# FederatedAI/FATE-LLM

Measured on AMD Instinct MI355X. Metric: GB/s param buffer reconstructed from (seed,scalar) list, device-resident, higher is better.
Workload: dtype bf16

## Files before the change

fate-llm_amd/csrc/fks_device.hip:

```cpp
#include <hip/hip_runtime.h>
#include <hip/hip_bf16.h>

#include <atomic>
#include <type_traits>
#include <mutex>

#include "fks_internal.h"
#include "fks_bitslice.h"
#define FKS_HD __device__ __forceinline__
#include "fks_libm.h"

constexpr int kDbMinWaves = 4;
constexpr int kZrUnroll = 2;
constexpr int kSm2MinWaves = 8;
constexpr int kBsFence = 8;
#ifndef FKS_BS_LAG
#define FKS_BS_LAG 36
#endif
#ifndef FKS_F32_SEED_PAIRS
#define FKS_F32_SEED_PAIRS 0
#endif
#ifndef FKS_LOG_INTMASK
#define FKS_LOG_INTMASK 1
#endif
#ifndef FKS_F32_TRIM
#define FKS_F32_TRIM 1
#endif

namespace fks {
namespace {

__device__ __forceinline__ uint32_t mt_twist(uint32_t u, uint32_t v) {
  return (((u & 0x80000000u) | (v & 0x7fffffffu)) >> 1) ^ ((v & 1u) ? kMatrixA : 0u);
}

constexpr unsigned kXorAnd = 0x78;
constexpr unsigned kXorMask = 0x28;
constexpr unsigned kXorNotAnd = 0xD2;

__device__ __forceinline__ uint32_t mt_temper(uint32_t y) {
  y ^= (y >> 11);
  y = __builtin_amdgcn_bitop3_b32(y, y << 7, 0x9d2c5680u, kXorAnd);
  y = __builtin_amdgcn_bitop3_b32(y, y << 15, 0xefc60000u, kXorAnd);
  y ^= (y >> 18);
  return y;
}


typedef __bf16 bf16x2_t __attribute__((ext_vector_type(2)));
typedef float f32x2_t __attribute__((ext_vector_type(2)));
__device__ __forceinline__ float rbf_cvt(float x) {
  const f32x2_t v = {0.0f, x};
  return __builtin_bit_cast(float, __builtin_convertvector(v, bf16x2_t));
}
__device__ __forceinline__ float rbf(float x) { return rbf_cvt(x); }
__device__ __forceinline__ float rhf(float x) {
  asm volatile("" : "+v"(x));
  return static_cast<float>(static_cast<_Float16>(x));
}

__device__ __forceinline__ uint32_t swap_adjacent(uint32_t v) {
  return (uint32_t)__builtin_amdgcn_mov_dpp((int)v, 0xB1, 0xF, 0xF, false);
}

__device__ __forceinline__ float cephes_logf(float x) {
#if FKS_LOG_INTMASK
  const uint32_t xb0 = __float_as_uint(x);
  const uint32_t xb = (xb0 & ~0x7f800000u) | 0x3f000000u;
  const int32_t m = (int32_t)(xb - 0x3F3504F3u) >> 31;
  const float e = (float)((int32_t)(xb0 >> 23) - 126 + m);
  const float tmp = __uint_as_float(xb & (uint32_t)m);
  x = __uint_as_float(xb) - 1.0f;
#else
  int32_t imm0 = (int32_t)(__float_as_uint(x) >> 23);
  x = __uint_as_float((__float_as_uint(x) & ~0x7f800000u) | 0x3f000000u);
  imm0 -= 0x7f;
  float e = (float)imm0;
  e = e + 1.0f;
  const bool mask = x < 0.707106781186547524f;
  const float tmp = mask ? x : 0.0f;
  x = x - 1.0f;
  e = e - (mask ? 1.0f : 0.0f);
#endif
  x = x + tmp;
  const float z = x * x;
  float y = 7.0376836292E-2f;
  y = __fmaf_rn(y, x, -1.1514610310E-1f);
  y = __fmaf_rn(y, x, 1.1676998740E-1f);
  y = __fmaf_rn(y, x, -1.2420140846E-1f);
  y = __fmaf_rn(y, x, +1.4249322787E-1f);
  y = __fmaf_rn(y, x, -1.6668057665E-1f);
  y = __fmaf_rn(y, x, +2.0000714765E-1f);
  y = __fmaf_rn(y, x, -2.4999993993E-1f);
  y = __fmaf_rn(y, x, +3.3333331174E-1f);
  y = y * x;
  y = __fmaf_rn(y, z, e * -2.12194440e-4f);
  y = __fmaf_rn(-z, 0.5f, y);
  x = x + y;
  x = __fmaf_rn(e, 0.693359375f, x);
  return x;
}


template <int DT>
struct Traits;

typedef __attribute__((address_space(1))) float gf32;
typedef __attribute__((address_space(1))) uint16_t gu16;
typedef __attribute__((address_space(1))) _Float16 gf16;

typedef __attribute__((address_space(1))) uint32_t gu32;

typedef __attribute__((address_space(1))) uint64_t gu64;

template <>
struct Traits<FKS_F32> {
  typedef uint64_t Pair;
  __device__ static Pair load_pair(uint64_t a) { return *reinterpret_cast<const gu64*>(a); }
  __device__ static void store_pair(uint64_t a, Pair v) { *reinterpret_cast<gu64*>(a) = v; }
  __device__ static uint32_t lo(Pair v) { return (uint32_t)v; }
  __device__ static uint32_t hi(Pair v) { return (uint32_t)(v >> 32); }
  __device__ static Pair pack(uint32_t l, uint32_t h) { return (uint64_t)l | ((uint64_t)h << 32); }
  __device__ static uint32_t bits(float v) { return __float_as_uint(v); }
  __device__ static uint32_t load_raw(uint64_t p, int64_t i) { return reinterpret_cast<const gu32*>(p)[i]; }
  __device__ static float cvt(uint32_t r) { return __uint_as_float(r); }
  __device__ static float load(uint64_t p, int64_t i) { return reinterpret_cast<const gf32*>(p)[i]; }
  __device__ static void store(uint64_t p, int64_t i, float v) { reinterpret_cast<gf32*>(p)[i] = v; }
  __device__ static float rnd(float x) { return x; }
};

template <>
struct Traits<FKS_BF16> {
  typedef uint32_t Pair;
  __device__ static Pair load_pair(uint64_t a) { return *reinterpret_cast<const gu32*>(a); }
  __device__ static void store_pair(uint64_t a, Pair v) { *reinterpret_cast<gu32*>(a) = v; }
  __device__ static uint32_t lo(Pair v) { return v & 0xffffu; }
  __device__ static uint32_t hi(Pair v) { return v >> 16; }
  __device__ static Pair pack(uint32_t l, uint32_t h) { return (l & 0xffffu) | (h << 16); }
  __device__ static uint32_t bits(float v) { return __float_as_uint(v) >> 16; }
  __device__ static uint32_t load_raw(uint64_t p, int64_t i) { return reinterpret_cast<const gu16*>(p)[i]; }
  __device__ static float cvt(uint32_t r) { return __uint_as_float(r << 16); }
  __device__ static float load(uint64_t p, int64_t i) {
    return __uint_as_float((uint32_t)reinterpret_cast<const gu16*>(p)[i] << 16);
  }
  __device__ static void store(uint64_t p, int64_t i, float v) {
    reinterpret_cast<gu16*>(p)[i] = (uint16_t)(__float_as_uint(v) >> 16);
  }
  __device__ static float rnd(float x) { return rbf(x); }
};

template <>
struct Traits<FKS_F16> {
  typedef uint32_t Pair;
  __device__ static Pair load_pair(uint64_t a) { return *reinterpret_cast<const gu32*>(a); }
  __device__ static void store_pair(uint64_t a, Pair v) { *reinterpret_cast<gu32*>(a) = v; }
  __device__ static uint32_t lo(Pair v) { return v & 0xffffu; }
  __device__ static uint32_t hi(Pair v) { return v >> 16; }
  __device__ static Pair pack(uint32_t l, uint32_t h) { return (l & 0xffffu) | (h << 16); }
  __device__ static uint32_t bits(float v) { return __builtin_bit_cast(uint16_t, static_cast<_Float16>(v)); }
  __device__ static uint32_t load_raw(uint64_t p, int64_t i) { return reinterpret_cast<const gu16*>(p)[i]; }
  __device__ static float cvt(uint32_t r) { return static_cast<float>(__builtin_bit_cast(_Float16, (uint16_t)r)); }
  __device__ static float load(uint64_t p, int64_t i) { return static_cast<float>(reinterpret_cast<const gf16*>(p)[i]); }
  __device__ static void store(uint64_t p, int64_t i, float v) { reinterpret_cast<gf16*>(p)[i] = static_cast<_Float16>(v); }
  __device__ static float rnd(float x) { return rhf(x); }
};

template <>
struct Traits<kDtF32Libm> : Traits<FKS_F32> {};
constexpr bool is_f32(int dt) { return dt == FKS_F32 || dt == kDtF32Libm; }

template <int DT>
__device__ __forceinline__ float apply_one(float p, float z, float g, float lr, float wd, bool has_wd, int mode,
                                           float ps, bool upd = true) {
  using TR = Traits<DT>;
  if (mode == kModeDelta) return __fmaf_rn(g, z, p);
  if (mode == kModePerturb || mode == kModePerturbUpdate) {
    p = TR::rnd(p + TR::rnd(ps * z));
    if (mode == kModePerturb || !upd) return p;
  }
  if (mode == kModeUpdate || mode == kModePerturbUpdate) {
    const float gz = TR::rnd(g * z);
    const float t2 = TR::rnd(gz + TR::rnd(wd * p));
    const float t = has_wd ? t2 : gz;
    return TR::rnd(p - TR::rnd(lr * t));
  }
  return z;
}

template <int DT>
__device__ __forceinline__ float dev_value_g(const float* v) {
  const float g = __int_as_float(__builtin_amdgcn_readfirstlane(__float_as_int(v[0])));
  return is_f32(DT) ? g : Traits<DT>::rnd(g);
}
__device__ __forceinline__ bool dev_value_apply(const float* v) {
  return __int_as_float(__builtin_amdgcn_readfirstlane(__float_as_int(v[1]))) != 0.0f;
}

constexpr int kJumpXOff = 3;

__device__ __forceinline__ void jump_quad_step10(uint32_t (&acc)[10], const uint32_t (&w)[13], uint32_t code) {
  asm volatile(
      "s_bitcmp1_b32 %[c], 3\n"
      "s_cbranch_scc1 .Lqb3k8x%=\n"
      "s_bitcmp1_b32 %[c], 2\n"
      "s_cbranch_scc1 .Lqb2k4x%=\n"
      "s_bitcmp1_b32 %[c], 1\n"
      "s_cbranch_scc1 .Lqb1k2x%=\n"
      "s_bitcmp1_b32 %[c], 0\n"
      "s_cbranch_scc1 .Lqb0k1x%=\n"
      "s_branch .Lqendx%=\n"
      ".Lqb0k1x%=:\n"
      "v_xor_b32 %[a0], %[a0], %[w0]\n"
      "v_xor_b32 %[a1], %[a1], %[w1]\n"
      "v_xor_b32 %[a2], %[a2], %[w2]\n"
      "v_xor_b32 %[a3], %[a3], %[w3]\n"
      "v_xor_b32 %[a4], %[a4], %[w4]\n"
      "v_xor_b32 %[a5], %[a5], %[w5]\n"
      "v_xor_b32 %[a6], %[a6], %[w6]\n"
      "v_xor_b32 %[a7], %[a7], %[w7]\n"
      "v_xor_b32 %[a8], %[a8], %[w8]\n"
      "v_xor_b32 %[a9], %[a9], %[w9]\n"
      "s_branch .Lqendx%=\n"
      ".Lqb1k2x%=:\n"
      "s_bitcmp1_b32 %[c], 0\n"
      "s_cbranch_scc1 .Lqb0k3x%=\n"
      "v_xor_b32 %[a0], %[a0], %[w1]\n"
      "v_xor_b32 %[a1], %[a1], %[w2]\n"
      "v_xor_b32 %[a2], %[a2], %[w3]\n"
      "v_xor_b32 %[a3], %[a3], %[w4]\n"
      "v_xor_b32 %[a4], %[a4], %[w5]\n"
      "v_xor_b32 %[a5], %[a5], %[w6]\n"
      "v_xor_b32 %[a6], %[a6], %[w7]\n"
      "v_xor_b32 %[a7], %[a7], %[w8]\n"
      "v_xor_b32 %[a8], %[a8], %[w9]\n"
      "v_xor_b32 %[a9], %[a9], %[w10]\n"
      "s_branch .Lqendx%=\n"
      ".Lqb0k3x%=:\n"
      "v_bitop3_b32 %[a0], %[a0], %[w0], %[w1] bitop3:0x96\n"
      "v_bitop3_b32 %[a1], %[a1], %[w1], %[w2] bitop3:0x96\n"
      "v_bitop3_b32 %[a2], %[a2], %[w2], %[w3] bitop3:0x96\n"
      "v_bitop3_b32 %[a3], %[a3], %[w3], %[w4] bitop3:0x96\n"
      "v_bitop3_b32 %[a4], %[a4], %[w4], %[w5] bitop3:0x96\n"
      "v_bitop3_b32 %[a5], %[a5], %[w5], %[w6] bitop3:0x96\n"
      "v_bitop3_b32 %[a6], %[a6], %[w6], %[w7] bitop3:0x96\n"
      "v_bitop3_b32 %[a7], %[a7], %[w7], %[w8] bitop3:0x96\n"
      "v_bitop3_b32 %[a8], %[a8], %[w8], %[w9] bitop3:0x96\n"
      "v_bitop3_b32 %[a9], %[a9], %[w9], %[w10] bitop3:0x96\n"
      "s_branch .Lqendx%=\n"
      ".Lqb2k4x%=:\n"
      "s_bitcmp1_b32 %[c], 1\n"
      "s_cbranch_scc1 .Lqb1k6x%=\n"
      "s_bitcmp1_b32 %[c], 0\n"
      "s_cbranch_scc1 .Lqb0k5x%=\n"
      "v_xor_b32 %[a0], %[a0], %[w2]\n"
      "v_xor_b32 %[a1], %[a1], %[w3]\n"
      "v_xor_b32 %[a2], %[a2], %[w4]\n"
      "v_xor_b32 %[a3], %[a3], %[w5]\n"
      "v_xor_b32 %[a4], %[a4], %[w6]\n"
      "v_xor_b32 %[a5], %[a5], %[w7]\n"
      "v_xor_b32 %[a6], %[a6], %[w8]\n"
      "v_xor_b32 %[a7], %[a7], %[w9]\n"
      "v_xor_b32 %[a8], %[a8], %[w10]\n"
      "v_xor_b32 %[a9], %[a9], %[w11]\n"
      "s_branch .Lqendx%=\n"
      ".Lqb0k5x%=:\n"
      "v_bitop3_b32 %[a0], %[a0], %[w0], %[w2] bitop3:0x96\n"
      "v_bitop3_b32 %[a1], %[a1], %[w1], %[w3] bitop3:0x96\n"
      "v_bitop3_b32 %[a2], %[a2], %[w2], %[w4] bitop3:0x96\n"
      "v_bitop3_b32 %[a3], %[a3], %[w3], %[w5] bitop3:0x96\n"
      "v_bitop3_b32 %[a4], %[a4], %[w4], %[w6] bitop3:0x96\n"
      "v_bitop3_b32 %[a5], %[a5], %[w5], %[w7] bitop3:0x96\n"
      "v_bitop3_b32 %[a6], %[a6], %[w6], %[w8] bitop3:0x96\n"
      "v_bitop3_b32 %[a7], %[a7], %[w7], %[w9] bitop3:0x96\n"
      "v_bitop3_b32 %[a8], %[a8], %[w8], %[w10] bitop3:0x96\n"
      "v_bitop3_b32 %[a9], %[a9], %[w9], %[w11] bitop3:0x96\n"
      "s_branch .Lqendx%=\n"
      ".Lqb1k6x%=:\n"
      "s_bitcmp1_b32 %[c], 0\n"
      "s_cbranch_scc1 .Lqb0k7x%=\n"
      "v_bitop3_b32 %[a0], %[a0], %[w1], %[w2] bitop3:0x96\n"
      "v_bitop3_b32 %[a1], %[a1], %[w2], %[w3] bitop3:0x96\n"
      "v_bitop3_b32 %[a2], %[a2], %[w3], %[w4] bitop3:0x96\n"
      "v_bitop3_b32 %[a3], %[a3], %[w4], %[w5] bitop3:0x96\n"
      "v_bitop3_b32 %[a4], %[a4], %[w5], %[w6] bitop3:0x96\n"
      "v_bitop3_b32 %[a5], %[a5], %[w6], %[w7] bitop3:0x96\n"
      "v_bitop3_b32 %[a6], %[a6], %[w7], %[w8] bitop3:0x96\n"
      "v_bitop3_b32 %[a7], %[a7], %[w8], %[w9] bitop3:0x96\n"
      "v_bitop3_b32 %[a8], %[a8], %[w9], %[w10] bitop3:0x96\n"
      "v_bitop3_b32 %[a9], %[a9], %[w10], %[w11] bitop3:0x96\n"
      "s_branch .Lqendx%=\n"
      ".Lqb0k7x%=:\n"
      "v_bitop3_b32 %[a0], %[a0], %[w0], %[w1] bitop3:0x96\n"
      "v_xor_b32 %[a0], %[a0], %[w2]\n"
      "v_bitop3_b32 %[a1], %[a1], %[w1], %[w2] bitop3:0x96\n"
      "v_xor_b32 %[a1], %[a1], %[w3]\n"
      "v_bitop3_b32 %[a2], %[a2], %[w2], %[w3] bitop3:0x96\n"
      "v_xor_b32 %[a2], %[a2], %[w4]\n"
      "v_bitop3_b32 %[a3], %[a3], %[w3], %[w4] bitop3:0x96\n"
      "v_xor_b32 %[a3], %[a3], %[w5]\n"
      "v_bitop3_b32 %[a4], %[a4], %[w4], %[w5] bitop3:0x96\n"
      "v_xor_b32 %[a4], %[a4], %[w6]\n"
      "v_bitop3_b32 %[a5], %[a5], %[w5], %[w6] bitop3:0x96\n"
      "v_xor_b32 %[a5], %[a5], %[w7]\n"
      "v_bitop3_b32 %[a6], %[a6], %[w6], %[w7] bitop3:0x96\n"
      "v_xor_b32 %[a6], %[a6], %[w8]\n"
      "v_bitop3_b32 %[a7], %[a7], %[w7], %[w8] bitop3:0x96\n"
      "v_xor_b32 %[a7], %[a7], %[w9]\n"
      "v_bitop3_b32 %[a8], %[a8], %[w8], %[w9] bitop3:0x96\n"
      "v_xor_b32 %[a8], %[a8], %[w10]\n"
      "v_bitop3_b32 %[a9], %[a9], %[w9], %[w10] bitop3:0x96\n"
      "v_xor_b32 %[a9], %[a9], %[w11]\n"
      "s_branch .Lqendx%=\n"
      ".Lqb3k8x%=:\n"
      "s_bitcmp1_b32 %[c], 2\n"
      "s_cbranch_scc1 .Lqb2k12x%=\n"
      "s_bitcmp1_b32 %[c], 1\n"
      "s_cbranch_scc1 .Lqb1k10x%=\n"
      "s_bitcmp1_b32 %[c], 0\n"
      "s_cbranch_scc1 .Lqb0k9x%=\n"
      "v_xor_b32 %[a0], %[a0], %[w3]\n"
// ... 1168 lines not shown
      u32x2_t w0, w1;
      w0.x = w.x;
      w0.y = w.y;
      w1.x = w.z;
      w1.y = w.w;
      zab = temper_pair_u8x8(w0);
      zcd = temper_pair_u8x8(w1);
      a.zidx[((size_t)(b0 + t - a.zlo)) * kZidxPerBlock + q] =
          (zab.x >> 3) | (zab.y << 5) | (zcd.x << 13) | (zcd.y << 21);
    }
    {
      if (sl.fast) {
        run(buf_c, sl.r0, sl.r1, u_lr, u_wd, u_wdf, u_ps);
        ST::store_pair(sl.base + joff, sl.r0);
        ST::store_pair(sl.base + joff + 8 * kEs, sl.r1);
      } else {
        const int64_t s1 = (int64_t)kMtN * (b0 + t) + j;
        int cc = sl.cur;
        bool in = false;
        DevSeg sg;
        while (cc < a.nsegs) {
          sg = a.segs[cc];
          if (s1 < sg.start + sg.numel) { in = s1 >= sg.start; break; }
          cc++;
        }
        if (in) {
          const uint64_t addr = sg.ptr + (uint64_t)(s1 - sg.start) * kEs;
          Pair r0 = 0, r1 = 0;
          if (MODE != kModeWriteZ) {
            r0 = ST::load_pair(addr);
            r1 = ST::load_pair(addr + 8 * kEs);
          }
          run(buf_c, r0, r1, sg.lr, sg.wd, (sg.flags & FKS_HAS_WD) != 0, sg.ps);
          ST::store_pair(addr, r0);
          ST::store_pair(addr + 8 * kEs, r1);
        }
      }
    }
    __syncthreads();
  };

  Slot s0 = fetch(0);
  *reinterpret_cast<volatile uint32_t*>(a.sink + 1) = 0u;
  for (int t = 0; t < nblk; t += 2) {
    Slot s1 = fetch(t + 1 < nblk ? t + 1 : t);
    block(std::integral_constant<int, 0>{}, s0, t);
    if (t + 1 >= nblk) break;
    s0 = fetch(t + 2 < nblk ? t + 2 : t + 1);
    block(std::integral_constant<int, 1>{}, s1, t + 1);
  }
}

constexpr int kZrThreads = 256;
typedef __attribute__((address_space(1))) u32x4_t gu32x4_t;
__device__ __forceinline__ u32x4_t gload4(uint64_t addr) { return *reinterpret_cast<const gu32x4_t*>(addr); }
__device__ __forceinline__ void gstore4(uint64_t addr, u32x4_t v) { *reinterpret_cast<gu32x4_t*>(addr) = v; }
constexpr int kZrTile = kZrThreads * 8;

template <int MODE>
__global__ __launch_bounds__(kZrThreads) void fks_zreplay_kernel(ApplyArgs a) {
  extern __shared__ __attribute__((aligned(16))) uint32_t lds32[];
  if ((uint32_t)(size_t)(lds_u32_t*)lds32 != 0u) __builtin_trap();
  const int tid = threadIdx.x;
  const int c = blockIdx.x;
  for (int i = tid; i < 256; i += kZrThreads) {
    reinterpret_cast<float*>(lds32)[i] = c_tab_bf16[i];
    reinterpret_cast<float*>(lds32)[256 + i] = c_tab_bf16[256 + i];
    reinterpret_cast<float*>(lds32)[512 + i] = c_tab_bf16[512 + i];
  }
  __syncthreads();
  const int64_t p0 = (int64_t)kMtN * a.chunk_block[0] + (int64_t)c * kZrTile;
  const int64_t p1 = (int64_t)kMtN * a.chunk_block[a.nchunks];
  const int64_t tstep = (int64_t)gridDim.x * kZrTile;
  const int64_t zbase = (int64_t)kMtN * a.zlo;
  const uint64_t zb = (uint64_t)(uintptr_t)a.zidx;
  float g = rflf(a.g[0]);
  bool upd = true;
  if (MODE == kModePerturbUpdate && a.gdev) {
    g = dev_value_g<FKS_BF16>(a.gdev);
    upd = dev_value_apply(a.gdev);
  }
  const uint32_t half = (uint32_t)tid & 1u;
  const uint32_t cs_tab = half ? 2048u : 1024u;

  int cur = 0;
  {
    int lo = 0, hi = a.nsegs;
    while (lo < hi) {
      const int mid = (lo + hi) >> 1;
      const DevSeg& sm = a.segs[mid];
      if ((int64_t)rfl64((uint64_t)(sm.start + sm.numel)) <= p0) lo = mid + 1; else hi = mid;
    }
    cur = lo;
  }
  auto chain = [&](u32x4_t pv, u32x4_t rec, float lr, float wd, bool wdf, float ps) __attribute__((always_inline)) -> u32x4_t {
    const uint32_t w[4] = {pv.x, pv.y, pv.z, pv.w};
    const uint32_t r[4] = {rec.x, rec.y, rec.z, rec.w};
    uint32_t o[4];
#pragma unroll
    for (int m = 0; m < 4; m++) {
      const uint32_t ri = r[m];
      const float ra = lds_f32((ri << 2) & 0x3FCu), rb = lds_f32((ri >> 14) & 0x3FCu);
      const float ca = lds_f32(cs_tab + ((ri >> 6) & 0x3FCu)), cb = lds_f32(cs_tab + ((ri >> 22) & 0x3FCu));
      const f32x2_t rr = {ra, rb}, cc = {ca, cb}, zero = {0.0f, 0.0f};
      const f32x2_t z = rnd2<FKS_BF16>(__builtin_elementwise_fma(rr, cc, zero));
      f32x2_t pe = {__uint_as_float(w[m] << 16), __uint_as_float(w[m] & 0xffff0000u)};
      pe = apply_pair<FKS_BF16, MODE>(pe, z, g, lr, wd, wdf, ps, upd);
      o[m] = __builtin_amdgcn_perm(__float_as_uint(pe.y), __float_as_uint(pe.x), 0x07060302u);
    }
    const u32x4_t out = {o[0], o[1], o[2], o[3]};
    return out;
  };
  const u32x4_t zero4 = {0u, 0u, 0u, 0u};
  struct ZSlot { int64_t t0; uint64_t base; float lr, wd, ps; int cur; bool fast, wdf; u32x4_t rec, pv; };
  int64_t seg_st = INT64_MAX, seg_en = INT64_MAX;
  uint64_t seg_ptr = 0;
  float seg_lr = 0.0f, seg_wd = 0.0f, seg_ps = 0.0f;
  bool seg_wdf = false;
  auto load_seg = [&]() __attribute__((always_inline)) {
    if (cur < a.nsegs) {
      const DevSeg& sg = a.segs[cur];
      seg_st = (int64_t)rfl64((uint64_t)sg.start);
      seg_en = seg_st + (int64_t)rfl64((uint64_t)sg.numel);
      seg_ptr = rfl64(sg.ptr);
      seg_lr = rflf(sg.lr);
      seg_wd = rflf(sg.wd);
      seg_ps = rflf(sg.ps);
      seg_wdf = (rfl(sg.flags) & FKS_HAS_WD) != 0;
    } else {
      seg_st = seg_en = INT64_MAX;
    }
  };
  load_seg();
  auto zfetch = [&](int64_t t0) __attribute__((always_inline)) -> ZSlot {
    ZSlot z;
    z.t0 = t0;
    while (seg_en <= t0) {
      cur++;
      load_seg();
    }
    z.cur = cur;
    const int64_t tend = t0 + kZrTile < p1 ? t0 + kZrTile : p1;
    z.fast = seg_st <= t0 && tend <= seg_en;
    z.base = seg_ptr + (uint64_t)(t0 - seg_st) * 2u;
    z.lr = seg_lr;
    z.wd = seg_wd;
    z.ps = seg_ps;
    z.wdf = seg_wdf;
    const int64_t pos = t0 + 8 * (int64_t)tid;
    const bool live = pos < p1;
    z.rec = zero4;
    z.pv = zero4;
    if (t0 < p1) {
      z.rec = gload4(zb + (uint64_t)(((live ? pos : t0) - zbase) & ~(int64_t)15));
      if (MODE != kModeWriteZ && z.fast) z.pv = gload4(z.base + (live ? 16u * (uint32_t)tid : 0u));
    }
    return z;
  };
  auto zblock = [&](ZSlot& z) __attribute__((always_inline)) {
    const int64_t pos = z.t0 + 8 * (int64_t)tid;
    if (pos >= p1) return;
    if (z.fast) {
      gstore4(z.base + 16u * (uint32_t)tid, chain(z.pv, z.rec, z.lr, z.wd, z.wdf, z.ps));
    } else {
      int cc = z.cur;
      bool in = false;
      DevSeg sg;
      while (cc < a.nsegs) {
        sg = a.segs[cc];
        if (pos < sg.start + sg.numel) { in = pos >= sg.start; break; }
        cc++;
      }
      if (in) {
        const uint64_t ptr = sg.ptr + (uint64_t)(pos - sg.start) * 2u;
        const u32x4_t pv = MODE == kModeWriteZ ? zero4 : gload4(ptr);
        gstore4(ptr, chain(pv, z.rec, sg.lr, sg.wd, (sg.flags & FKS_HAS_WD) != 0, sg.ps));
      }
    }
  };
  constexpr int kU = kZrUnroll;
  for (int64_t t0 = p0; t0 < p1; t0 += kU * tstep) {
    ZSlot z[kU];
#pragma unroll
    for (int u = 0; u < kU; u++) z[u] = zfetch(t0 + u * tstep);
#pragma unroll
    for (int u = 0; u < kU; u++) zblock(z[u]);
  }
}

constexpr int kBsChunkBytes = kMtN * 16;
constexpr int kBsStateBytes = 8 * kBsChunkBytes;
constexpr int kBsTabBytes = 256 * 4 + 256 * 8;
constexpr uint32_t kBsFlagOff = kBsTabBytes + 2 * kBsStateBytes;
constexpr uint32_t kBsProgOff = kBsFlagOff + 8;
constexpr uint32_t kBsProg1Off = kBsProgOff + 4 * 6;
constexpr int kBsLdsBytes = (int)kBsProg1Off + 4 * 6;
static_assert(kBsLdsBytes <= 163840, "slice kernel LDS");
constexpr int kBsWaves = kBsHalfThreads / 64;
constexpr int kBsTaskWords = 128;

__device__ __forceinline__ void bs_store_row(uint32_t ra, const uint32_t (&x)[32]) {
#pragma unroll
  for (int q = 0; q < 8; q++) {
    const u32x4_t v = {x[4 * q], x[4 * q + 1], x[4 * q + 2], x[4 * q + 3]};
    lds_st4(ra + q * kBsChunkBytes, v);
  }
}

__device__ __forceinline__ uint32_t bs_flag_load(uint32_t off) {
  return *(volatile const lds_u32_t*)(size_t)off;
}
__device__ __forceinline__ void bs_flag_store(uint32_t off, uint32_t v) {
  asm volatile("" ::: "memory");
  __builtin_amdgcn_s_waitcnt(0xC07F);
  *(volatile lds_u32_t*)(size_t)off = v;
}

template <int S>
__device__ __forceinline__ uint32_t bs_index(uint32_t w, int c) {
  switch (c) {
    case 0: return bs::byte_x<0, S>(w);
    case 1: return bs::byte_x<1, S>(w);
    case 2: return bs::byte_x<2, S>(w);
    default: return bs::byte_x<3, S>(w);
  }
}

#if FKS_BS_WGTIME
__device__ uint64_t g_bs_wgtime[4096][16];
extern "C" int fks_debug_bs_wgtime(uint64_t* out, int nblocks) {
  return (int)hipMemcpyFromSymbol(out, HIP_SYMBOL(g_bs_wgtime), sizeof(uint64_t) * 16 * (size_t)nblocks, 0,
                                  hipMemcpyDeviceToHost);
}
#endif

template <int MODE, bool FULL>
__global__ __launch_bounds__(kBsThreads, 1) void fks_apply_bs_kernel(ApplyBsArgs a) {
  extern __shared__ __attribute__((aligned(16))) uint32_t lds32[];
  if ((uint32_t)(size_t)(lds_u32_t*)lds32 != 0u) __builtin_trap();
  const int tid = threadIdx.x;
  const int lane = tid & 63;
#if FKS_BS_WGTIME
  if (tid == 0) g_bs_wgtime[blockIdx.x][0] = __builtin_amdgcn_s_memrealtime();
  auto stamp = [&]() { if (lane == 0) g_bs_wgtime[blockIdx.x][1 + (tid >> 6)] = __builtin_amdgcn_s_memrealtime(); };
#else
  auto stamp = [&]() {};
#endif
  const int half = __builtin_amdgcn_readfirstlane(tid >= kBsHalfThreads ? 1 : 0);
  const int ht = tid - half * kBsHalfThreads;
  const int hw = __builtin_amdgcn_readfirstlane(ht >> 6);
  const bool split = a.split != 0;
  const int c = split ? 2 * (int)blockIdx.x + half : (int)blockIdx.x;
  const int nA = FULL ? kBsSeeds : split ? a.nseeds : (a.nseeds + 1) / 2;
  const int nseeds = FULL ? kBsSeeds : (half && !split ? a.nseeds - nA : nA);
  const int sfirst = half && !split ? nA : 0;
  const int64_t b0 = a.chunk_block[split ? c : 2 * c], b1 = a.chunk_block[split ? c + 1 : 2 * c + 2];
  const int nwords = (int)(kMtN * (b1 - b0));
  const int ntask = (nwords + kBsTaskWords - 1) / kBsTaskWords;
  const uint32_t sbase = kBsTabBytes + (uint32_t)half * kBsStateBytes;
  const uint32_t flag = kBsFlagOff + 4u * (uint32_t)half;

  for (int i = tid; i < 256; i += kBsThreads) {
    reinterpret_cast<float*>((uint8_t*)lds32)[i] = c_tab_bf16[i];
    reinterpret_cast<float2*>((uint8_t*)lds32 + 1024)[i] = make_float2(c_tab_bf16[256 + i], c_tab_bf16[512 + i]);
  }
  for (int i = ht; i < kMtN; i += kBsHalfThreads) {
    uint32_t w[32];
#pragma unroll
    for (int k = 0; k < 32; k++)
      w[k] = k < nseeds ? a.states[((size_t)(a.use_slot ? a.slot[sfirst + k] : (uint32_t)(sfirst + k)) * a.nchunks + c) *
                                       kMtN + i]
                        : 0u;
    bs::transpose32(w);
    bs_store_row(sbase + 16u * (uint32_t)i, w);
  }
  if (ht == 0) lds32[flag / 4] = 0u;
  if (ht < kBsWaves) lds32[(half ? kBsProg1Off : kBsProgOff) / 4 + ht] = 0u;
  __syncthreads();
  if (nseeds == 0) return;

  const int toff = 16 * (lane >> 3) + (lane & 7);
  const bool flip = ((lane >> 3) & 1) != 0;
  const bool odd = (lane & 1) != 0;

  float gk[kBsSeeds];
#pragma unroll
  for (int k = 0; k < kBsSeeds; k++) gk[k] = a.g[half ? k + sfirst : k];

  const int64_t wbase = (int64_t)kMtN * b0;
  int cur;
  {
    const int64_t s1 = wbase + (int64_t)kBsTaskWords * hw + toff;
    int lo = 0, hi = a.nsegs;
    while (lo < hi) {
      const int mid = (lo + hi) >> 1;
      if (a.segs[mid].start + a.segs[mid].numel <= s1) lo = mid + 1; else hi = mid;
    }
    cur = lo;
  }
  int64_t seg_start = INT64_MAX, seg_end = INT64_MAX;
  uint64_t seg_ptr = 0;
  float seg_lr = 0.0f, seg_wd = 0.0f;
  bool seg_wdf = false;
  auto load_seg = [&]() {
    if (cur < a.nsegs) {
      const DevSeg sg = a.segs[cur];
      seg_start = sg.start;
      seg_end = sg.start + sg.numel;
      seg_ptr = sg.ptr;
      seg_lr = sg.lr;
      seg_wd = sg.wd;
      seg_wdf = (sg.flags & FKS_HAS_WD) != 0;
    } else {
      seg_start = seg_end = INT64_MAX;
    }
    __builtin_amdgcn_s_waitcnt(0x0F70);
  };
  load_seg();

  using ST = Traits<MODE == kModeDelta ? FKS_F32 : FKS_BF16>;
  constexpr int kEs = MODE == kModeDelta ? 4 : 2;
  typedef typename ST::Pair Pair;
  struct Slot { uint64_t addr; float lr, wd; uint32_t wdf; Pair raw; };
  auto fetch = [&](int n) -> Slot {
    Slot sl;
    const int u1 = kBsTaskWords * n + toff;
    const int64_t s1 = wbase + u1;
    while (s1 >= seg_end) { cur++; load_seg(); }
    const bool on = u1 < nwords && s1 >= seg_start;
    sl.lr = seg_lr; sl.wd = seg_wd; sl.wdf = seg_wdf;
    sl.addr = on ? seg_ptr + (uint64_t)(s1 - seg_start + (odd ? 7 : 0)) * kEs : (uint64_t)(uintptr_t)a.sink;
    sl.raw = ST::load_pair(sl.addr);
    return sl;
  };

  auto twist = [&](const int n, uint32_t (&oa)[8], uint32_t (&ob)[8]) {
    const int u1 = kBsTaskWords * n + toff;
    const bool valid = u1 < nwords;
    const int i1 = valid ? u1 % kMtN : 0;
    const int ia = flip ? i1 + 8 : i1, ib = flip ? i1 : i1 + 8;
    auto rows = [&](int i, uint32_t& av, uint32_t& am, uint32_t& au) {
      const int iv = i + 1 < kMtN ? i + 1 : 0;
      const int im = i < kMtN - kMtM ? i + kMtM : i - (kMtN - kMtM);
      av = sbase + 16u * (uint32_t)iv;
      am = sbase + 16u * (uint32_t)im;
      au = sbase + 7u * kBsChunkBytes + 16u * (uint32_t)i + 12u;
    };
    uint32_t av1, am1, au1, av2, am2, au2;
    rows(ia, av1, am1, au1);
    rows(ib, av2, am2, au2);
    uint32_t M1[32], M2[32];
    const uint32_t U1 = lds_u32((int)au1), U2 = lds_u32((int)au2);
    u32x4_t va = lds_u4(av1), vb = lds_u4(av2), ma = lds_u4(am1), mb = lds_u4(am2);
    const uint32_t v0a = va.x, v0b = vb.x;
#pragma unroll
    for (int q = 0; q < 8; q++) {
      u32x4_t va2 = va, vb2 = vb, ma2 = ma, mb2 = mb;
      if (q < 7) {
        va2 = lds_u4(av1 + (q + 1) * kBsChunkBytes);
        vb2 = lds_u4(av2 + (q + 1) * kBsChunkBytes);
        ma2 = lds_u4(am1 + (q + 1) * kBsChunkBytes);
        mb2 = lds_u4(am2 + (q + 1) * kBsChunkBytes);
      }
      const uint32_t Va[5] = {va.x, va.y, va.z, va.w, va2.x};
      const uint32_t Vb[5] = {vb.x, vb.y, vb.z, vb.w, vb2.x};
      const uint32_t Ma[4] = {ma.x, ma.y, ma.z, ma.w}, Mb[4] = {mb.x, mb.y, mb.z, mb.w};
#pragma unroll
      for (int t = 0; t < 4; t++) {
        const int b = 4 * q + t;
        const bool am = ((bs::kMatrixA >> b) & 1u) != 0;
        uint32_t xa, xb;
        if (b < 30) { xa = Va[t + 1]; xb = Vb[t + 1]; }
        else if (b == 30) { xa = U1; xb = U2; }
        else { xa = 0u; xb = 0u; }
        M1[b] = am ? bs::xor3(Ma[t], xa, v0a) : (Ma[t] ^ xa);
        M2[b] = am ? bs::xor3(Mb[t], xb, v0b) : (Mb[t] ^ xb);
      }
      if (valid) {
        lds_st4(sbase + 16u * (uint32_t)ia + q * kBsChunkBytes, u32x4_t{M1[4 * q], M1[4 * q + 1], M1[4 * q + 2], M1[4 * q + 3]});
        lds_st4(sbase + 16u * (uint32_t)ib + q * kBsChunkBytes, u32x4_t{M2[4 * q], M2[4 * q + 1], M2[4 * q + 2], M2[4 * q + 3]});
      }
      va = va2; vb = vb2; ma = ma2; mb = mb2;
    }
    uint32_t o1[8], o2[8];
    bs::temper_low8(M1, o1);
    bs::temper_low8(M2, o2);
#pragma unroll
    for (int j = 0; j < 8; j++) {
      oa[j] = flip ? o2[j] : o1[j];
      ob[j] = flip ? o1[j] : o2[j];
    }
  };

  auto chain = [&](const Slot& sl, uint32_t (&oa)[8], uint32_t (&ob)[8]) {
    bs::transpose8(oa);
    bs::transpose8(ob);
    f32x2_t p;
    {
      const uint32_t keep = odd ? ST::hi(sl.raw) : ST::lo(sl.raw);
      const uint32_t got = swap_adjacent(odd ? ST::lo(sl.raw) : ST::hi(sl.raw));
      p.x = ST::cvt(odd ? got : keep);
      p.y = ST::cvt(odd ? keep : got);
    }
    auto z_of = [&](const int k) __attribute__((always_inline)) -> f32x2_t {
      const float r = lds_f32(bs_index<2>(oa[k & 7], k >> 3));
      const f32x2_t rr = {r, r}, zero = {0.0f, 0.0f};
      const f32x2_t cs = lds_f32x2(1024u + bs_index<3>(ob[k & 7], k >> 3));
      return rnd2<FKS_BF16>(__builtin_elementwise_fma(rr, cs, zero));
    };
    {
#pragma unroll
      for (int k = 0; k < kBsSeeds; k++) {
        if (FULL || k < nseeds) p = apply_pair<FKS_BF16, MODE>(p, z_of(k), gk[k], sl.lr, sl.wd, sl.wdf != 0, 0.0f);
        if ((k % kBsFence) == kBsFence - 1) asm volatile("" ::: "memory");
      }
    }
    const uint32_t b1v = ST::bits(p.x), b2v = ST::bits(p.y);
    const uint32_t back = swap_adjacent(odd ? b1v : b2v);
    const Pair out = odd ? ST::pack(back, b2v) : ST::pack(b1v, back);
    ST::store_pair(sl.addr, out);
  };

  const bool ordered = !split;
  const uint32_t prog = kBsProgOff + 4u * (uint32_t)hw;
  auto publish_stored = [&](const int m) {
    asm volatile("" ::: "memory");
    __builtin_amdgcn_s_waitcnt(0x0F70);
    if (lane == 0) *(volatile lds_u32_t*)(size_t)prog = (uint32_t)m + 1u;
  };
  auto await_stored = [&](const int m) {
    if (m >= ntask) return;
    const uint32_t pm = kBsProgOff + 4u * (uint32_t)(m % kBsWaves);
    while (__builtin_amdgcn_readfirstlane(bs_flag_load(pm)) < (uint32_t)m + 1u) __builtin_amdgcn_s_sleep(1);
    asm volatile("" ::: "memory");
  };
  static_assert(FKS_BS_LAG == 0 || FKS_BS_LAG > 2 * kBsWaves, "FKS_BS_LAG: half 1 trails by 12 tasks");
  constexpr bool kLag = FKS_BS_LAG > 0 && (MODE == kModeUpdateWd || MODE == kModeUpdate);
  const uint32_t prog1 = kBsProg1Off + 4u * (uint32_t)hw;
  auto publish_applied = [&](const int m) {
    if (lane == 0) *(volatile lds_u32_t*)(size_t)prog1 = (uint32_t)m + 1u;
  };
  auto await_applied = [&](const int m) {
    if (m < 0) return;
    const uint32_t pm = kBsProg1Off + 4u * (uint32_t)(m % kBsWaves);
    while (__builtin_amdgcn_readfirstlane(bs_flag_load(pm)) < (uint32_t)m + 1u) __builtin_amdgcn_s_sleep(1);
  };

  auto task = [&](const int n, const Slot& sl, Slot& nx) {
    uint32_t oa[8], ob[8];
    if (kLag && ordered && half == 0) await_applied(n - FKS_BS_LAG);
    __builtin_amdgcn_s_setprio(2);
#if !FKS_BS_DIAG_NOWAIT
    while (__builtin_amdgcn_readfirstlane(bs_flag_load(flag)) < (uint32_t)n) __builtin_amdgcn_s_sleep(0);
#endif
    asm volatile("" ::: "memory");
    twist(n, oa, ob);
    if (lane == 0) bs_flag_store(flag, (uint32_t)n + 1u);
    __builtin_amdgcn_s_setprio(0);
    if (ordered && half == 0) {
      if (n >= kBsWaves) publish_stored(n - kBsWaves);
    } else if (ordered) {
      await_stored(n + kBsWaves);
    }
    nx = fetch(n + kBsWaves);
#if FKS_BS_DIAG_NOCHAIN
    if (__builtin_amdgcn_readfirstlane(oa[0] ^ ob[0]) == 0x12345u) chain(sl, oa, ob);
#else
    chain(sl, oa, ob);
#endif
    if (kLag && ordered && half) publish_applied(n);
  };

  if (hw >= ntask) { stamp(); return; }
  if (ordered && half) await_stored(hw);
  Slot s0 = fetch(hw), s1;
  int n = hw;
  for (;;) {
    task(n, s0, s1);
    if (n + kBsWaves >= ntask) break;
    n += kBsWaves;
    task(n, s1, s0);
    if (n + kBsWaves >= ntask) break;
    n += kBsWaves;
  }
  if (ordered && half == 0) publish_stored(n);
  stamp();
}

__constant__ float c_tab_f16[3 * 2048];

constexpr int kIrrCarry = 16;
constexpr int kIrrWin = kIrrCarry + kMtN;

__device__ __forceinline__ uint32_t win_word(const uint32_t* win, int k, int w) {
  return win[k * kIrrWin + kIrrCarry + w];
}

template <int PH>
__device__ __forceinline__ void irr_twist_phase(uint32_t* win, int nseeds, int tid) {
  constexpr int lo = PH == 0 ? 0 : (PH == 1 ? 227 : 454);
  constexpr int hi = PH == 0 ? 227 : (PH == 1 ? 454 : kMtN);
  constexpr int len = hi - lo;
  constexpr int per = (kMaxSeedsPerPass * len + kApplyThreads - 1) / kApplyThreads;
  uint32_t v[per];
#pragma unroll
  for (int j = 0; j < per; j++) {
    const int idx = tid + j * kApplyThreads;
    if (idx < nseeds * len) {
      const int k = idx / len, i = lo + idx % len;
      const uint32_t* w = win + k * kIrrWin + kIrrCarry;
      const uint32_t nx = i == kMtN - 1 ? w[0] : w[i + 1];
      const uint32_t m = i < kMtN - kMtM ? w[i + kMtM] : w[i - (kMtN - kMtM)];
      v[j] = m ^ mt_twist(w[i], nx);
    }
  }
  uint32_t cv = 0;
  if (PH == 0 && tid < nseeds * kIrrCarry) cv = win[(tid / kIrrCarry) * kIrrWin + kIrrCarry + kMtN - kIrrCarry + tid % kIrrCarry];
  __syncthreads();
#pragma unroll
  for (int j = 0; j < per; j++) {
    const int idx = tid + j * kApplyThreads;
    if (idx < nseeds * len) win[(idx / len) * kIrrWin + kIrrCarry + lo + idx % len] = v[j];
  }
  if (PH == 0 && tid < nseeds * kIrrCarry) win[(tid / kIrrCarry) * kIrrWin + tid % kIrrCarry] = cv;
  __syncthreads();
}

constexpr int kIrrLogfOff = kLdsTabBytes + 4 * (kIrrWin * kMaxSeedsPerPass + 16);
static_assert(kIrrLogfOff % 16 == 0, "logf table alignment");

template <int DT>
__device__ __forceinline__ void irr_z_pair(const uint8_t* lds, uint32_t r1, uint32_t r2, float& z1, float& z2) {
  if constexpr (DT == kDtF32Libm) {
    z_pair_f32_libm((uint32_t)kIrrLogfOff, r1, r2, z1, z2);
  } else if constexpr (DT == FKS_F16) {
    const uint32_t a = mt_temper(r1) & 0x7FFu, b = mt_temper(r2) & 0x7FFu;
    z1 = rhf(__fmaf_rn(c_tab_f16[a], c_tab_f16[2048 + b], 0.0f));
    z2 = rhf(__fmaf_rn(c_tab_f16[a], c_tab_f16[4096 + b], 0.0f));
  } else {
    z_pair<DT>(lds, r1, r2, z1, z2);
  }
}

template <int DT, int MODE>
__device__ __forceinline__ void irr_run_lane(const uint8_t* lds, const uint32_t* win, const IrrArgs& a, const DevRun& R,
                                             int64_t e1, int w1) {
  using TR = Traits<MODE == kModeDelta ? FKS_F32 : DT>;
  const bool on1 = e1 < R.limit, on2 = e1 + 8 < R.limit;
  float p1 = 0.0f, p2 = 0.0f;
  if (MODE != kModeWriteZ) {
    if (on1) p1 = TR::load(R.ptr, e1);
    if (on2) p2 = TR::load(R.ptr, e1 + 8);
  }
  const bool has_wd = (R.flags & FKS_HAS_WD) != 0;
  const float* g = a.g[DT == kDtF32Libm ? FKS_F32 : DT];
  const bool dv = MODE == kModePerturbUpdate && a.gdev;
  const bool upd = dv ? dev_value_apply(a.gdev) : true;
  for (int k = 0; k < a.nseeds; k++) {
    float z1, z2;
    irr_z_pair<DT>(lds, win_word(win, k, w1), win_word(win, k, w1 + 8), z1, z2);
    const float gv = dv ? dev_value_g<DT>(a.gdev) : g[k];
    p1 = apply_one<DT>(p1, z1, gv, R.lr, R.wd, has_wd, MODE, R.ps, upd);
    p2 = apply_one<DT>(p2, z2, gv, R.lr, R.wd, has_wd, MODE, R.ps, upd);
  }
  if (on1) TR::store(R.ptr, e1, p1);
  if (on2) TR::store(R.ptr, e1 + 8, p2);
}

__device__ __forceinline__ double u53(uint32_t hi, uint32_t lo) {
  const uint64_t x = (((uint64_t)hi << 32) | lo) & ((1ull << 53) - 1);
  return (double)x * (1.0 / 9007199254740992.0);
}

template <int DT, int MODE>
__device__ __forceinline__ void irr_tiny_lane(const uint32_t* win, const IrrArgs& a, const DevTiny& T, int w) {
  using TR = Traits<MODE == kModeDelta ? FKS_F32 : DT>;
  float p = MODE != kModeWriteZ ? TR::load(T.ptr, 0) : 0.0f;
  const bool has_wd = (T.flags & FKS_HAS_WD) != 0;
  const bool sin_half = (T.flags & kTinySin) != 0;
  const float* g = a.g[DT];
  const bool dv = MODE == kModePerturbUpdate && a.gdev;
  const bool upd = dv ? dev_value_apply(a.gdev) : true;
  for (int k = 0; k < a.nseeds; k++) {
    const double u1 = u53(mt_temper(win_word(win, k, w)), mt_temper(win_word(win, k, w + 1)));
    const double u2 = u53(mt_temper(win_word(win, k, w + 2)), mt_temper(win_word(win, k, w + 3)));
    const double r = sqrt(-2.0 * fks_libm::log1p(-u2));
    const double theta = 2.0 * 3.14159265358979323846 * u1;
    const double v = r * fks_libm::sin_or_cos(theta, sin_half) * 1.0 + 0.0;
    const float zf = (float)v;
    const float z = DT == FKS_F32 ? zf : Traits<DT>::rnd(zf);
    p = apply_one<DT>(p, z, dv ? dev_value_g<DT>(a.gdev) : g[k], T.lr, T.wd, has_wd, MODE, T.ps, upd);
  }
  TR::store(T.ptr, 0, p);
}

template <int MODE>
__global__ __launch_bounds__(kApplyThreads) void fks_irregular_kernel(IrrArgs a) {
  extern __shared__ __attribute__((aligned(16))) uint32_t lds32[];
  uint8_t* lds = reinterpret_cast<uint8_t*>(lds32);
  uint32_t* win = reinterpret_cast<uint32_t*>(lds + kLdsTabBytes);
  uint32_t* cnt = win + kIrrWin * kMaxSeedsPerPass;
  if ((uint32_t)(size_t)(lds_u32_t*)lds32 != 0u) __builtin_trap();
  const int tid = threadIdx.x;
  const int c = blockIdx.x;
  const int nseeds = a.nseeds;
  const int64_t b0 = a.chunk_lo[c], b1 = a.chunk_hi[c];
  {
    float2* tabCS = reinterpret_cast<float2*>(lds + kLdsCsOff);
    for (int i = tid; i < 256; i += kApplyThreads) {
      reinterpret_cast<float*>(lds)[i] = c_tab_bf16[i];
      tabCS[i] = make_float2(c_tab_bf16[256 + i], c_tab_bf16[512 + i]);
    }
  }
  if (a.libm) logf_tab_fill((uint32_t)kIrrLogfOff, tid, kApplyThreads);
  for (int idx = tid; idx < nseeds * kMtN; idx += kApplyThreads) {
    const int k = idx / kMtN, i = idx - k * kMtN;
    win[k * kIrrWin + kIrrCarry + i] = a.states[((size_t)k * a.nchunks + c) * kMtN + i];
  }
  int ri, ti;
  {
    int lo = 0, hi = a.nruns;
    while (lo < hi) {
      const int mid = (lo + hi) >> 1;
      if (a.runs[mid].start + a.runs[mid].numel - 1 < (int64_t)kMtN * b0) lo = mid + 1; else hi = mid;
    }
    ri = lo;
    lo = 0, hi = a.ntiny;
    while (lo < hi) {
      const int mid = (lo + hi) >> 1;
      if (a.tiny[mid].word + 3 < (int64_t)kMtN * b0) lo = mid + 1; else hi = mid;
    }
    ti = lo;
  }
  __syncthreads();
  const int m = tid >> 3, r8 = tid & 7;
  for (int64_t b = b0; b < b1; b++) {
    irr_twist_phase<0>(win, nseeds, tid);
    irr_twist_phase<1>(win, nseeds, tid);
    irr_twist_phase<2>(win, nseeds, tid);
    const int64_t base = (int64_t)kMtN * b, end = base + kMtN;
    while (ri < a.nruns && a.runs[ri].start + 15 < end) {
      const DevRun R = a.runs[ri];
      const int ph = (int)(R.start & 15);
      const int64_t s0 = base + 16 * m + (ph ? ph - 16 : 0);
      if (tid < kMtN / 2 && s0 >= R.start && s0 < R.start + R.numel) {
        const int64_t e1 = s0 - R.start + r8;
        const int w1 = (int)(s0 - base) + r8;
        switch (R.dtype) {
          case FKS_F32:
            if (a.libm) irr_run_lane<kDtF32Libm, MODE>(lds, win, a, R, e1, w1);
            else irr_run_lane<FKS_F32, MODE>(lds, win, a, R, e1, w1);
            break;
          case FKS_BF16: irr_run_lane<FKS_BF16, MODE>(lds, win, a, R, e1, w1); break;
          default: irr_run_lane<FKS_F16, MODE>(lds, win, a, R, e1, w1); break;
        }
      }
      if (R.start + R.numel - 1 < end) ri++; else break;
    }
    for (;;) {
      const int idx = ti + tid;
      const bool mine = idx < a.ntiny && a.tiny[idx].word + 3 < end;
      if (mine) {
        const DevTiny T = a.tiny[idx];
        const int w = (int)(T.word - base);
        switch (T.dtype) {
          case FKS_F32: irr_tiny_lane<FKS_F32, MODE>(win, a, T, w); break;
          case FKS_BF16: irr_tiny_lane<FKS_BF16, MODE>(win, a, T, w); break;
          default: irr_tiny_lane<FKS_F16, MODE>(win, a, T, w); break;
        }
      }
      const uint64_t bal = __ballot(mine);
      if ((tid & 63) == 0) cnt[tid >> 6] = (uint32_t)__popcll(bal);
      __syncthreads();
      int n = 0;
#pragma unroll
      for (int w = 0; w < kApplyThreads / 64; w++) n += (int)cnt[w];
      __syncthreads();
      ti += n;
      if (n < kApplyThreads) break;
    }
  }
}

struct PhxRound1 {
  uint32_t a0, a2;
  uint32_t c1, c3;
};
__device__ __forceinline__ PhxRound1 philox_round1(uint64_t ctr, uint32_t idx) {
  const uint64_t m0 = (uint64_t)0xD2511F53u * (uint32_t)ctr, m1 = (uint64_t)0xCD9E8D57u * idx;
  return PhxRound1{(uint32_t)(m1 >> 32) ^ (uint32_t)(ctr >> 32), (uint32_t)(m0 >> 32), (uint32_t)m1, (uint32_t)m0};
}
__device__ __forceinline__ uint4 philox4x32_10(const PhxRound1& r1, uint64_t seed) {
  uint32_t k0 = (uint32_t)seed, k1 = (uint32_t)(seed >> 32);
  uint32_t c0 = r1.a0 ^ k0, c1 = r1.c1, c2 = r1.a2 ^ k1, c3 = r1.c3;
  k0 += 0x9E3779B9u;
  k1 += 0xBB67AE85u;
#pragma unroll
  for (int r = 1; r < 10; r++) {
    const uint64_t m0 = (uint64_t)0xD2511F53u * c0, m1 = (uint64_t)0xCD9E8D57u * c2;
    const uint32_t n0 = bs::xor3((uint32_t)(m1 >> 32), c1, k0), n2 = bs::xor3((uint32_t)(m0 >> 32), c3, k1);
    c1 = (uint32_t)m1;
    c3 = (uint32_t)m0;
    c0 = n0;
    c2 = n2;
    k0 += 0x9E3779B9u;
    k1 += 0xBB67AE85u;
  }
  return make_uint4(c0, c1, c2, c3);
}

__device__ __forceinline__ float2 rocrand_box_muller(uint32_t x, uint32_t y) {
  const float u = __fmaf_rn((float)x, 2.3283064e-10f, 2.3283064e-10f);
  const float v = __fmaf_rn((float)y, 1.46291807e-09f, 1.46291807e-09f);
  const float s = sqrtf(-2.0f * logf(u));
  float sn, cs;
  __sincosf(v, &sn, &cs);
  return make_float2(__fmaf_rn(sn * s, 1.0f, 0.0f), __fmaf_rn(cs * s, 1.0f, 0.0f));
}

template <int DT>
__device__ __forceinline__ float phx_cast(float v) {
  return DT == FKS_F32 ? v : Traits<DT>::rnd(v);
}

constexpr uint32_t kPhxFastUlps = 2;
__device__ __forceinline__ f32x2_t phx_radius2_fast(const f32x2_t u) {
  const f32x2_t y = {__builtin_amdgcn_logf(u.x), __builtin_amdgcn_logf(u.y)};
  const f32x2_t x = y * (f32x2_t){__uint_as_float(0xbfb17218u), __uint_as_float(0xbfb17218u)};
  return (f32x2_t){__builtin_amdgcn_sqrtf(x.x), __builtin_amdgcn_sqrtf(x.y)};
}

template <bool kExact = true>
__device__ __forceinline__ f32x2_t phx_radius2(const f32x2_t u) {
  const f32x2_t y = {__builtin_amdgcn_logf(u.x), __builtin_amdgcn_logf(u.y)};
  const f32x2_t m2hi = {__uint_as_float(0xbfb17217u), __uint_as_float(0xbfb17217u)};
  const f32x2_t m2lo = {__uint_as_float(0xb3f7d1cfu), __uint_as_float(0xb3f7d1cfu)};
  const f32x2_t r = y * m2hi;
  f32x2_t e = __builtin_elementwise_fma(y, m2hi, -r);
  e = __builtin_elementwise_fma(m2lo, y, e);
  const f32x2_t x = r + e;
  f32x2_t sq = {__builtin_amdgcn_sqrtf(x.x), __builtin_amdgcn_sqrtf(x.y)};
  if (!kExact) return sq;
  const f32x2_t sm = {__int_as_float(__float_as_int(sq.x) - 1), __int_as_float(__float_as_int(sq.y) - 1)};
  const f32x2_t sp = {__int_as_float(__float_as_int(sq.x) + 1), __int_as_float(__float_as_int(sq.y) + 1)};
  const f32x2_t rm = __builtin_elementwise_fma(-sm, sq, x), rp = __builtin_elementwise_fma(-sp, sq, x);
  sq.x = rm.x <= 0.0f ? sm.x : sq.x;
  sq.y = rm.y <= 0.0f ? sm.y : sq.y;
  sq.x = rp.x > 0.0f ? sp.x : sq.x;
  sq.y = rp.y > 0.0f ? sp.y : sq.y;
  return sq;
}

template <bool kExact = true, bool kFast = false>
__device__ __forceinline__ void phx_box_muller2(const uint4 w, f32x2_t& zA, f32x2_t& zB) {
  const f32x2_t cu = {2.3283064e-10f, 2.3283064e-10f}, cv = {1.46291807e-09f, 1.46291807e-09f};
  const f32x2_t fx = {(float)w.x, (float)w.z}, fy = {(float)w.y, (float)w.w};
  const f32x2_t u = __builtin_elementwise_fma(fx, cu, cu);
  const f32x2_t sq = kFast ? phx_radius2_fast(u) : phx_radius2<kExact>(u);
  const f32x2_t v = __builtin_elementwise_fma(fy, cv, cv);
  const f32x2_t rev = v * (f32x2_t){__uint_as_float(0x3e22f983u), __uint_as_float(0x3e22f983u)};
  const f32x2_t sc1 = {__builtin_amdgcn_sinf(rev.x), __builtin_amdgcn_cosf(rev.x)};
  const f32x2_t sc2 = {__builtin_amdgcn_sinf(rev.y), __builtin_amdgcn_cosf(rev.y)};
  const f32x2_t zero = {0.0f, 0.0f};
  zA = __builtin_elementwise_fma(sc1, (f32x2_t){sq.x, sq.x}, zero);
  zB = __builtin_elementwise_fma(sc2, (f32x2_t){sq.y, sq.y}, zero);
}

#ifndef FKS_PHX_FAST_LOG
#define FKS_PHX_FAST_LOG 1
#endif
constexpr uint32_t kPhxMidW = FKS_PHX_FAST_LOG ? 2 * kPhxFastUlps + 2 : 4;
__device__ __forceinline__ bool phx_near_bf16_mid(float z) {
  return ((__float_as_uint(z) & 0xFFFFu) - (0x8000u - kPhxMidW)) <= 2 * kPhxMidW;
}
__device__ __forceinline__ void phx_z_bf16(const uint4 w, f32x2_t& zA, f32x2_t& zB) {
#if FKS_PHX_EXACT_RADIUS
  phx_box_muller2<true>(w, zA, zB);
#else
  phx_box_muller2<false, FKS_PHX_FAST_LOG != 0>(w, zA, zB);
  const bool near = (int)phx_near_bf16_mid(zA.x) | (int)phx_near_bf16_mid(zA.y) | (int)phx_near_bf16_mid(zB.x) |
                    (int)phx_near_bf16_mid(zB.y);
  if (__builtin_expect(near, 0)) phx_box_muller2<true>(w, zA, zB);
#endif
  zA = rnd2<FKS_BF16>(zA);
  zB = rnd2<FKS_BF16>(zB);
}
// ... 637 lines not shown
```

Baseline: 1.253.

## Offload part of radius-table lookups to global memory and strength-reduce row indexing

For the update-without-weight-decay mode, some of the per-seed radius table reads (the first FKS_BS_R_VMEM of every 8) now come from a global constant table via vector memory instead of LDS, issued early before the fetch. The aim is to relieve LDS bandwidth pressure in the bitsliced chain. Segment bounds are precomputed as 32-bit offsets relative to the block base so fetch avoids 64-bit compares. The MT row index is advanced incrementally rather than computed with a modulo. The gathered global loads add VMEM latency and cache pressure and raise register use.

Result: faster. 1.279, median of 6 (+2.1%).

```diff
diff --git a/fate-llm_amd/csrc/fks_device.hip b/fate-llm_amd/csrc/fks_device.hip
--- a/fate-llm_amd/csrc/fks_device.hip
+++ b/fate-llm_amd/csrc/fks_device.hip
@@ -16,6 +16,9 @@
 constexpr int kBsFence = 8;
 #ifndef FKS_BS_LAG
 #define FKS_BS_LAG 36
+#endif
+#ifndef FKS_BS_R_VMEM
+#define FKS_BS_R_VMEM 3
 #endif
 #ifndef FKS_F32_SEED_PAIRS
 #define FKS_F32_SEED_PAIRS 0
@@ -1790,6 +1793,10 @@
   uint64_t seg_ptr = 0;
   float seg_lr = 0.0f, seg_wd = 0.0f;
   bool seg_wdf = false;
+  constexpr int kEs = MODE == kModeDelta ? 4 : 2;
+  constexpr bool kInc = MODE == kModeUpdateWd0;
+  int seg_lo = INT32_MAX, seg_hi = INT32_MAX;
+  uint64_t seg_org = 0;
   auto load_seg = [&]() {
     if (cur < a.nsegs) {
       const DevSeg sg = a.segs[cur];
@@ -1802,30 +1809,49 @@
     } else {
       seg_start = seg_end = INT64_MAX;
     }
+    if (kInc) {
+      const int64_t lo = seg_start - wbase, hi = seg_end - wbase;
+      seg_lo = (int)(lo < INT32_MIN ? INT32_MIN : lo > INT32_MAX ? INT32_MAX : lo);
+      seg_hi = (int)(hi < INT32_MIN ? INT32_MIN : hi > INT32_MAX ? INT32_MAX : hi);
+      seg_org = seg_ptr - (uint64_t)lo * kEs;
+    }
     __builtin_amdgcn_s_waitcnt(0x0F70);
   };
   load_seg();
 
   using ST = Traits<MODE == kModeDelta ? FKS_F32 : FKS_BF16>;
-  constexpr int kEs = MODE == kModeDelta ? 4 : 2;
   typedef typename ST::Pair Pair;
   struct Slot { uint64_t addr; float lr, wd; uint32_t wdf; Pair raw; };
   auto fetch = [&](int n) -> Slot {
     Slot sl;
     const int u1 = kBsTaskWords * n + toff;
-    const int64_t s1 = wbase + u1;
-    while (s1 >= seg_end) { cur++; load_seg(); }
-    const bool on = u1 < nwords && s1 >= seg_start;
-    sl.lr = seg_lr; sl.wd = seg_wd; sl.wdf = seg_wdf;
-    sl.addr = on ? seg_ptr + (uint64_t)(s1 - seg_start + (odd ? 7 : 0)) * kEs : (uint64_t)(uintptr_t)a.sink;
+    if (kInc) {
+      while (u1 >= seg_hi) { cur++; load_seg(); }
+      const bool on = u1 < nwords && u1 >= seg_lo;
+      sl.lr = seg_lr; sl.wd = seg_wd; sl.wdf = seg_wdf;
+      sl.addr = on ? seg_org + (uint64_t)(uint32_t)(u1 + (odd ? 7 : 0)) * kEs : (uint64_t)(uintptr_t)a.sink;
+    } else {
+      const int64_t s1 = wbase + u1;
+      while (s1 >= seg_end) { cur++; load_seg(); }
+      const bool on = u1 < nwords && s1 >= seg_start;
+      sl.lr = seg_lr; sl.wd = seg_wd; sl.wdf = seg_wdf;
+      sl.addr = on ? seg_ptr + (uint64_t)(s1 - seg_start + (odd ? 7 : 0)) * kEs : (uint64_t)(uintptr_t)a.sink;
+    }
     sl.raw = ST::load_pair(sl.addr);
     return sl;
   };
 
+  constexpr int kRowStep = kBsWaves * kBsTaskWords % kMtN;
+  int row = (kBsTaskWords * hw + toff) % kMtN;
+  auto next_row = [&]() {
+    if (!kInc) return;
+    row += kRowStep;
+    if (row >= kMtN) row -= kMtN;
+  };
   auto twist = [&](const int n, uint32_t (&oa)[8], uint32_t (&ob)[8]) {
     const int u1 = kBsTaskWords * n + toff;
     const bool valid = u1 < nwords;
-    const int i1 = valid ? u1 % kMtN : 0;
+    const int i1 = valid ? (kInc ? row : u1 % kMtN) : 0;
     const int ia = flip ? i1 + 8 : i1, ib = flip ? i1 : i1 + 8;
     auto rows = [&](int i, uint32_t& av, uint32_t& am, uint32_t& au) {
       const int iv = i + 1 < kMtN ? i + 1 : 0;
@@ -1880,9 +1906,25 @@
     }
   };
 
-  auto chain = [&](const Slot& sl, uint32_t (&oa)[8], uint32_t (&ob)[8]) {
+  constexpr int kRv = kInc ? FKS_BS_R_VMEM : 0;
+  static_assert(kRv >= 0 && kRv <= 8, "FKS_BS_R_VMEM");
+  auto rv_slot = [](const int k) __attribute__((always_inline)) -> int {
+    return (k & 7) < kRv ? (k >> 3) * kRv + (k & 7) : -1;
+  };
+  auto chain_head = [&](uint32_t (&oa)[8], uint32_t (&ob)[8], float (&rv)[4 * kRv + 1]) {
     bs::transpose8(oa);
     bs::transpose8(ob);
+#pragma unroll
+    for (int k = 0; k < kBsSeeds; k++)
+      if (rv_slot(k) >= 0)
+        rv[rv_slot(k)] =
+            *reinterpret_cast<const float*>(reinterpret_cast<const char*>(c_tab_bf16) + bs_index<2>(oa[k & 7], k >> 3));
+  };
+  auto chain = [&](const Slot& sl, uint32_t (&oa)[8], uint32_t (&ob)[8], const float (&rv)[4 * kRv + 1]) {
+    if (kRv == 0) {
+      bs::transpose8(oa);
+      bs::transpose8(ob);
+    }
     f32x2_t p;
     {
       const uint32_t keep = odd ? ST::hi(sl.raw) : ST::lo(sl.raw);
@@ -1891,7 +1933,7 @@
       p.y = ST::cvt(odd ? keep : got);
     }
     auto z_of = [&](const int k) __attribute__((always_inline)) -> f32x2_t {
-      const float r = lds_f32(bs_index<2>(oa[k & 7], k >> 3));
+      const float r = rv_slot(k) >= 0 ? rv[rv_slot(k)] : lds_f32(bs_index<2>(oa[k & 7], k >> 3));
       const f32x2_t rr = {r, r}, zero = {0.0f, 0.0f};
       const f32x2_t cs = lds_f32x2(1024u + bs_index<3>(ob[k & 7], k >> 3));
       return rnd2<FKS_BF16>(__builtin_elementwise_fma(rr, cs, zero));
@@ -1950,11 +1992,13 @@
     } else if (ordered) {
       await_stored(n + kBsWaves);
     }
+    float rv[4 * kRv + 1];
+    if (kRv > 0) chain_head(oa, ob, rv);
     nx = fetch(n + kBsWaves);
 #if FKS_BS_DIAG_NOCHAIN
-    if (__builtin_amdgcn_readfirstlane(oa[0] ^ ob[0]) == 0x12345u) chain(sl, oa, ob);
+    if (__builtin_amdgcn_readfirstlane(oa[0] ^ ob[0]) == 0x12345u) chain(sl, oa, ob, rv);
 #else
-    chain(sl, oa, ob);
+    chain(sl, oa, ob, rv);
 #endif
     if (kLag && ordered && half) publish_applied(n);
   };
@@ -1967,9 +2011,11 @@
     task(n, s0, s1);
     if (n + kBsWaves >= ntask) break;
     n += kBsWaves;
+    next_row();
     task(n, s1, s0);
     if (n + kBsWaves >= ntask) break;
     n += kBsWaves;
+    next_row();
   }
   if (ordered && half == 0) publish_stored(n);
   stamp();
```
